# HpWang-whu/YOHO

Hardware: AMD Instinct MI355X
Metric: keypoints/sec (5000 kp x60 rot desc+YOHO-O) (higher is better)
Workload: dtype fp16x2 split (2^-22-accurate products, fp32 accumulate); 1 GPU

## Files before the change

### yoho_amd/csrc/gemmf2.hip

```cpp
#include <hip/hip_runtime.h>
#include <cstdlib>
#include <cstring>
#include "common.h"
#include "gemmf.h"

namespace yoho {

constexpr int F2_BUF = 24576;
constexpr int F2_LDS = 3 * F2_BUF;
constexpr int F3_BUF = 32768;
constexpr int F3_LDS = 3 * F3_BUF;

struct Frags2 {
    uintx4 ah[4], al[4], bh[2], bl[2];
};

template <int LO, int R>
__device__ __forceinline__ void read_frag2(const char* pa, const char* pb, Frags2& f) {
    if constexpr (R < 4) f.al[R] = *reinterpret_cast<const uintx4*>(pa + 8192 + R * 512);
    else if constexpr (R < 6) f.bh[R - 4] = *reinterpret_cast<const uintx4*>(pb + (R - 4) * 512);
    else if constexpr (R < 10) f.ah[R - 6] = *reinterpret_cast<const uintx4*>(pa + (R - 6) * 512);
    else f.bl[R - 10] = *reinterpret_cast<const uintx4*>(pb + LO + (R - 10) * 512);
}
template <int LO>
__device__ __forceinline__ void read_frags2(const char* pa, const char* pb, Frags2& f) {
    sfor<0, 12>([&](auto rc) { read_frag2<LO, decltype(rc)::value>(pa, pb, f); });
}

struct Dma2 {
    static constexpr int NP = 6, LO = 4096;
    int la, lb, w;
    __device__ __forceinline__ Dma2(int w_, int lane) : la(w_ * 1024 + lane * 16), lb((w_ >> 1) * 4096 + (w_ & 1) * 1024 + lane * 16), w(w_) {}
    template <int U>
    __device__ __forceinline__ void piece(const char* srcA, const char* srcB, char* buf) const {
        if constexpr (U < 4) {
            constexpr int plane = U >> 1, kg = U & 1;
            __builtin_amdgcn_global_load_lds((gptr_t)(srcA + plane * 16384 + kg * 4096 + la), (lptr_t)(buf + plane * 8192 + kg * 4096 + w * 1024), 16, 0, 0);
        } else {
            constexpr int plane = U - 4;
            __builtin_amdgcn_global_load_lds((gptr_t)(srcB + plane * 16384 + lb), (lptr_t)(buf + 16384 + plane * 4096 + (w >> 1) * 2048 + (w & 1) * 1024), 16, 0, 0);
        }
    }
};
struct Dma3 {
    static constexpr int NP = 4, LO = 8192;
    int la, ldst;
    __device__ __forceinline__ Dma3(int w8, int lane) : la(w8 * 1024 + lane * 16), ldst(w8 * 1024) {}
    template <int U>
    __device__ __forceinline__ void piece(const char* srcA, const char* srcB, char* buf) const {
        constexpr int plane = U & 1;
        if constexpr (U < 2) __builtin_amdgcn_global_load_lds((gptr_t)(srcA + plane * 16384 + la), (lptr_t)(buf + plane * 8192 + ldst), 16, 0, 0);
        else __builtin_amdgcn_global_load_lds((gptr_t)(srcB + plane * 16384 + la), (lptr_t)(buf + 16384 + plane * 8192 + ldst), 16, 0, 0);
    }
};
template <typename Dma>
__device__ __forceinline__ void dma_step(const Dma& dm, const char* srcA, const char* srcB, char* buf) {
    sfor<0, Dma::NP>([&](auto uc) { dm.template piece<decltype(uc)::value>(srcA, srcB, buf); });
}

template <bool DMA, typename Dma>
__device__ __forceinline__ void step2(const Dma& dm, const Frags2& f, floatx16 (&acc)[4][2], const char* ra, const char* rb, Frags2& nf,
                                      const char* srcA, const char* srcB, char* dmabuf) {
    sfor<0, 8>([&](auto gc) {
        constexpr int g = decltype(gc)::value;
        acc[g >> 1][g & 1] = mfma_h(f.al[g >> 1], f.bh[g & 1], acc[g >> 1][g & 1]);
        read_frag2<Dma::LO, g>(ra, rb, nf);
        __builtin_amdgcn_sched_barrier(0);
    });
    sfor<0, 8>([&](auto gc) {
        constexpr int g = decltype(gc)::value;
        acc[g >> 1][g & 1] = mfma_h(f.ah[g >> 1], f.bl[g & 1], acc[g >> 1][g & 1]);
        if constexpr (g < 4) read_frag2<Dma::LO, 8 + g>(ra, rb, nf);
        else if constexpr (DMA) dm.template piece<g - 4>(srcA, srcB, dmabuf);
        __builtin_amdgcn_sched_barrier(0);
    });
    sfor<0, 8>([&](auto gc) {
        constexpr int g = decltype(gc)::value;
        acc[g >> 1][g & 1] = mfma_h(f.ah[g >> 1], f.bh[g & 1], acc[g >> 1][g & 1]);
        if constexpr (DMA && 4 + g < Dma::NP) dm.template piece<4 + g>(srcA, srcB, dmabuf);
        __builtin_amdgcn_sched_barrier(0);
    });
}

__host__ __device__ inline bool fg2_map(const FGemmArgs& a, int xcd, int slot, bool contiguous, int& t, int& local, int& r) {
    int cnt[NIR_ORD], ru[NIR_ORD];
    for (int u = 0; u < NIR_ORD; ++u) {
        ru[u] = (xcd + a.rot[u]) & 7;
        cnt[u] = a.NT[u] > ru[u] ? ((a.NT[u] - 1 - ru[u]) / 8 + 1) * a.MT[u] * 2 : 0;
    }
    const int L = cnt[0], S = cnt[1] + cnt[2] + cnt[3] + cnt[4];
    int list, idx;
    if (contiguous) { list = slot < L ? 0 : 1; idx = slot < L ? slot : slot - L; }
    else {
        const int P = L < S ? L : S;
        if (slot < 2 * P) { list = slot & 1; idx = slot >> 1; }
        else { list = L > S ? 0 : 1; idx = P + (slot - 2 * P); }
    }
    if (list == 0) {
        if (idx >= L) return false;
        t = 0; local = idx; r = ru[0];
        return true;
    }
    for (int u = 1; u < NIR_ORD; ++u) {
        if (idx < cnt[u]) { t = u; local = idx; r = ru[u]; return true; }
        idx -= cnt[u];
    }
    return false;
}

__device__ __forceinline__ size_t step_off(int ks) { return (size_t)(ks >> 1) * FG_STAGE + (size_t)(ks & 1) * 8192; }

template <int BUF, typename Dma>
__device__ __forceinline__ void ring_prologue(int KT, Dma&& dma) {
    dma(0, 0);
    dma(1, BUF);
    if (KT > 2) dma(2, 2 * BUF);
}

template <int BUF, int INFLIGHT, typename F, typename Step>
__device__ __forceinline__ void ring_pipelined(char* smem, const char* Ag, const char* Bg, int KT, int lane_a, int lane_b, F& P, Step&& step) {
    F Q;
    asm volatile("s_waitcnt lgkmcnt(0)" ::: "memory");
    __builtin_amdgcn_s_barrier();
    __builtin_amdgcn_sched_barrier(0);
    int cur = 0, nxt = BUF;
    int s = 0;
    auto run = [&](auto dma, const F& f, F& nf) {
        if constexpr (decltype(dma)::value) {
            step(dma, f, nf, smem + nxt + lane_a, smem + nxt + lane_b, uniform_ptr(Ag + step_off(s + 3)), uniform_ptr(Bg + step_off(s + 3)), smem + cur);
            asm volatile("s_waitcnt vmcnt(%0) lgkmcnt(0)" ::"n"(INFLIGHT) : "memory");
        } else {
            step(dma, f, nf, smem + nxt + lane_a, smem + nxt + lane_b, nullptr, nullptr, nullptr);
            asm volatile("s_waitcnt vmcnt(0) lgkmcnt(0)" ::: "memory");
        }
        __builtin_amdgcn_s_barrier();
        __builtin_amdgcn_sched_barrier(0);
        cur = nxt; nxt = nxt == 2 * BUF ? 0 : nxt + BUF; ++s;
    };
    constexpr std::true_type dma;
    constexpr std::false_type nodma;
    while (s + 4 < KT) {
        run(dma, P, Q);
        run(dma, Q, P);
    }
    if (KT >= 4) {
        run(dma, P, Q);
        run(nodma, Q, P);
    }
    run(nodma, P, Q);
    step(nodma, Q, P, smem + cur + lane_a, smem + cur + lane_b, nullptr, nullptr, nullptr);
}

template <int BUF, typename Dma>
__device__ __forceinline__ void ring_pipelined_idle(int KT, Dma&& dma) {
    __builtin_amdgcn_s_barrier();
    for (int s = 0; s + 1 < KT; ++s) {
        if (s + 3 < KT) dma(s + 3, (s % 3) * BUF);
        asm volatile("s_waitcnt vmcnt(0)" ::: "memory");
        __builtin_amdgcn_s_barrier();
    }
}

__global__ __launch_bounds__(256, 2) void fgemm2_kernel(FGemmArgs a, int flags) {
    extern __shared__ __attribute__((aligned(16))) char smem[];
    const int tid = threadIdx.x, lane = tid & 63;
    const int w = __builtin_amdgcn_readfirstlane(tid >> 6);
    int t = 0, local = 0, r = 0;
    if (!fg2_map(a, blockIdx.x & 7, blockIdx.x >> 3, (flags & F2_MIX) == 0, t, local, r)) return;
    const int d = a.dim[t];
    const int MT = a.MT[t], KS = d * a.cin / 32, KT = 2 * KS;
    const int nh = local & 1, pair = local >> 1;
    const int cg = pair / MT, mtile = pair - cg * MT;
    const int ntile = r + 8 * cg;
    const char* Ag = a.A + a.a_off[t] + (size_t)mtile * KS * FG_STAGE;
    const char* Bg = a.B + a.b_off[t] + (size_t)ntile * KS * FG_STAGE + nh * 2048;
    const int wm = w >> 1, wn = w & 1;
    const Dma2 dm(w, lane);
    const int lane_a = (lane >> 5) * 4096 + (wm * 128 + (lane & 31)) * 16;
    const int lane_b = 16384 + (lane >> 5) * 2048 + (wn * 64 + (lane & 31)) * 16;

    floatx16 acc[4][2];
    zero_acc(acc);
    auto dma = [&](int st, int buf) { dma_step(dm, Ag + step_off(st), Bg + step_off(st), smem + buf); };
    ring_prologue<F2_BUF>(KT, dma);
    const int row0 = mtile * 256 + wm * 128, colbase = ntile * 256 + nh * 128 + wn * 64;
    const bool rows_live = row0 < d * a.cout;
    const int jidx = colbase / a.kppad, kp0 = colbase - jidx * a.kppad, qbase = a.qbase[t];
    if ((flags & EPI_RES) && rows_live) residual_start(acc, row0, kp0, jidx, d, qbase, a.res, a.descale, a.cout, a.nT32, lane);
    asm volatile("s_waitcnt vmcnt(0)" ::: "memory");
    __builtin_amdgcn_s_barrier();
    if (!rows_live) return ring_pipelined_idle<F2_BUF>(KT, dma);

    Frags2 P;
    read_frags2<Dma2::LO>(smem + lane_a, smem + lane_b, P);
    ring_pipelined<F2_BUF, 6>(smem, Ag, Bg, KT, lane_a, lane_b, P,
        [&](auto dmac, const Frags2& f, Frags2& nf, const char* ra, const char* rb, const char* srcA, const char* srcB, char* buf) {
            step2<decltype(dmac)::value>(dm, f, acc, ra, rb, nf, srcA, srcB, buf);
        });
    coef_epilogue(acc, row0, kp0, jidx, d, qbase, a.out, a.bias, a.descale, a.cout, a.nT32, a.rflag, lane, flags);
}

struct Wave3 {
    int wm, wn, nh, lane_a, lane_b;
    Dma3 dm;
    __device__ __forceinline__ Wave3(int w8, int lane) : wm((w8 & 3) >> 1), wn(w8 & 1), nh(w8 >> 2), dm(w8, lane) {
        lane_a = (lane >> 5) * 4096 + (wm * 128 + (lane & 31)) * 16;
        lane_b = 16384 + (lane >> 5) * 4096 + (nh * 128 + wn * 64 + (lane & 31)) * 16;
    }
};

__global__ __launch_bounds__(512, 2) void fgemm3_kernel(FGemmArgs a, int flags) {
    extern __shared__ __attribute__((aligned(16))) char smem[];
    const int tid = threadIdx.x, lane = tid & 63;
    const Wave3 wv(__builtin_amdgcn_readfirstlane(tid >> 6), lane);
    int t = 0, local = 0, r = 0;
    if (!fg3_map(a, blockIdx.x & 7, blockIdx.x >> 3, t, local, r)) return;
    const int d = a.dim[t];
    const int MT = a.MT[t], KS = d * a.cin / 32, KT = 2 * KS;
    const int cg = local / MT, mtile = local - cg * MT;
    const int ntile = r + 8 * cg;
    const char* Ag = a.A + a.a_off[t] + (size_t)mtile * KS * FG_STAGE;
    const char* Bg = a.B + a.b_off[t] + (size_t)ntile * KS * FG_STAGE;

    floatx16 acc[4][2];
    zero_acc(acc);
    auto dma = [&](int st, int buf) { dma_step(wv.dm, Ag + step_off(st), Bg + step_off(st), smem + buf); };
    ring_prologue<F3_BUF>(KT, dma);
    const int row0 = mtile * 256 + wv.wm * 128, colbase = ntile * 256 + wv.nh * 128 + wv.wn * 64;
    const bool rows_live = row0 < d * a.cout;
    const int jidx = colbase / a.kppad, kp0 = colbase - jidx * a.kppad, qbase = a.qbase[t];
    if ((flags & EPI_RES) && rows_live) residual_start(acc, row0, kp0, jidx, d, qbase, a.res, a.descale, a.cout, a.nT32, lane);
    asm volatile("s_waitcnt vmcnt(0)" ::: "memory");
    __builtin_amdgcn_s_barrier();
    if (!rows_live) return ring_pipelined_idle<F3_BUF>(KT, dma);

    Frags2 P;
    read_frags2<Dma3::LO>(smem + wv.lane_a, smem + wv.lane_b, P);
    ring_pipelined<F3_BUF, 4>(smem, Ag, Bg, KT, wv.lane_a, wv.lane_b, P,
        [&](auto dmac, const Frags2& f, Frags2& nf, const char* ra, const char* rb, const char* srcA, const char* srcB, char* buf) {
            step2<decltype(dmac)::value>(wv.dm, f, acc, ra, rb, nf, srcA, srcB, buf);
        });
    coef_epilogue(acc, row0, kp0, jidx, d, qbase, a.out, a.bias, a.descale, a.cout, a.nT32, a.rflag, lane, flags);
}

constexpr int F3K_BUF = 2 * FG_STAGE;
constexpr int F3K_LDS = 2 * F3K_BUF;

struct Dma3k {
    static constexpr int NP = 8;
    int la, ldst;
    __device__ __forceinline__ Dma3k(int w8, int lane) : la(w8 * 1024 + lane * 16), ldst(w8 * 1024) {}
    template <int U>
    __device__ __forceinline__ void piece(const char* srcA, const char* srcB, char* buf) const {
        constexpr int q = (U & 3) * 8192;
        if constexpr (U < 4) __builtin_amdgcn_global_load_lds((gptr_t)(srcA + q + la), (lptr_t)(buf + q + ldst), 16, 0, 0);
        else __builtin_amdgcn_global_load_lds((gptr_t)(srcB + q + la), (lptr_t)(buf + FG_STAGE + q + ldst), 16, 0, 0);
    }
};
struct FragsA32 { uintx4 al, ah; };
struct FragsB32 { uintx4 bh[4], bl[4]; };

template <int R>
__device__ __forceinline__ void read_open32(const char* pa, const char* pb, FragsA32& a0, FragsB32& b) {
    if constexpr (R == 0) a0.al = *reinterpret_cast<const uintx4*>(pa + 16384);
    else if constexpr (R < 5) b.bh[R - 1] = *reinterpret_cast<const uintx4*>(pb + (R - 1) * 256);
    else if constexpr (R == 5) a0.ah = *reinterpret_cast<const uintx4*>(pa);
    else b.bl[R - 6] = *reinterpret_cast<const uintx4*>(pb + 16384 + (R - 6) * 256);
}

template <bool DMA>
__device__ __forceinline__ void step32(const Dma3k& dm, floatx4 (&acc)[8][4], FragsA32 (&fa)[2], const FragsB32& b, FragsB32& nb, const char* pa,
                                       const char* npa, const char* npb, const char* srcA, const char* srcB, char* dmabuf) {
    sfor<0, 7>([&](auto ic) {
        constexpr int i = decltype(ic)::value;
        row_products32(acc[i], fa[i & 1].al, fa[i & 1].ah, b.bh, b.bl, [&](auto mc) {
            constexpr int m = decltype(mc)::value;
            if constexpr (m == 1) fa[(i + 1) & 1].al = *reinterpret_cast<const uintx4*>(pa + 16384 + (i + 1) * 256);
            if constexpr (m == 2) fa[(i + 1) & 1].ah = *reinterpret_cast<const uintx4*>(pa + (i + 1) * 256);
        });
    });
    asm volatile("s_waitcnt vmcnt(0) lgkmcnt(0)" ::: "memory");
    __builtin_amdgcn_s_barrier();
    __builtin_amdgcn_sched_barrier(0);
    row_products32(acc[7], fa[1].al, fa[1].ah, b.bh, b.bl, [&](auto mc) {
        constexpr int m = decltype(mc)::value;
        if constexpr (m < 5) {
            read_open32<2 * m>(npa, npb, fa[0], nb);
            read_open32<2 * m + 1>(npa, npb, fa[0], nb);
        }
        if constexpr (DMA && m >= 4) dm.template piece<m - 4>(srcA, srcB, dmabuf);
    });
}

__global__ __launch_bounds__(512, 2) void fgemm3k_kernel(FGemmArgs a, int flags) {
    extern __shared__ __attribute__((aligned(16))) char smem[];
    const int tid = threadIdx.x, lane = tid & 63;
    const int w8 = __builtin_amdgcn_readfirstlane(tid >> 6);
    int t = 0, local = 0, r = 0;
    if (!fg3_map(a, blockIdx.x & 7, blockIdx.x >> 3, t, local, r)) return;
    const int d = a.dim[t];
    const int MT = a.MT[t], KS = d * a.cin / 32;
    const int cg = local / MT, mtile = local - cg * MT;
    const int ntile = r + 8 * cg;
    const char* Ag = a.A + a.a_off[t] + (size_t)mtile * KS * FG_STAGE;
    const char* Bg = a.B + a.b_off[t] + (size_t)ntile * KS * FG_STAGE;
    const int wm = (w8 & 3) >> 1, wn = w8 & 1, nh = w8 >> 2;
    const Dma3k dm(w8, lane);
    const int lane_a = (lane >> 4) * 4096 + (wm * 128 + (lane & 15)) * 16;
    const int lane_b = FG_STAGE + (lane >> 4) * 4096 + (nh * 128 + wn * 64 + (lane & 15)) * 16;

    floatx4 acc[8][4];
    zero_acc(acc);
    auto dma = [&](int st, int buf) {
        const char* sa = uniform_ptr(Ag + (size_t)st * FG_STAGE);
        const char* sb = uniform_ptr(Bg + (size_t)st * FG_STAGE);
        sfor<0, Dma3k::NP>([&](auto uc) { dm.template piece<decltype(uc)::value>(sa, sb, smem + buf); });
    };
    dma(0, 0);
    if (KS > 1) dma(1, F3K_BUF);
    const int row0 = mtile * 256 + wm * 128, colbase = ntile * 256 + nh * 128 + wn * 64;
    const bool rows_live = row0 < d * a.cout;
    const int jidx = colbase / a.kppad, kp0 = colbase - jidx * a.kppad, qbase = a.qbase[t];
    if ((flags & EPI_RES) && rows_live) residual_start(acc, row0, kp0, jidx, d, qbase, a.res, a.descale, a.cout, a.nT32, lane);
    asm volatile("s_waitcnt vmcnt(0)" ::: "memory");
    __builtin_amdgcn_s_barrier();
    if (!rows_live) {
        for (int s = 0; s < KS; ++s) {
            asm volatile("s_waitcnt vmcnt(0)" ::: "memory");
            __builtin_amdgcn_s_barrier();
            if (s + 2 < KS) dma(s + 2, (s & 1) * F3K_BUF);
        }
        asm volatile("s_waitcnt vmcnt(0)" ::: "memory");
        return;
    }

    FragsA32 fa[2];
    FragsB32 P, Q;
    sfor<0, 10>([&](auto rc) { read_open32<decltype(rc)::value>(smem + lane_a, smem + lane_b, fa[0], P); });
    int s = 0, cur = 0;
    auto run = [&](auto dmac, const FragsB32& b, FragsB32& nb) {
        const int nxt = cur ^ F3K_BUF;
        if constexpr (decltype(dmac)::value)
            step32<true>(dm, acc, fa, b, nb, smem + cur + lane_a, smem + nxt + lane_a, smem + nxt + lane_b, uniform_ptr(Ag + (size_t)(s + 2) * FG_STAGE),
                         uniform_ptr(Bg + (size_t)(s + 2) * FG_STAGE), smem + cur);
        else
            step32<false>(dm, acc, fa, b, nb, smem + cur + lane_a, smem + nxt + lane_a, smem + nxt + lane_b, nullptr, nullptr, nullptr);
        cur = nxt; ++s;
    };
    constexpr std::true_type dmay;
    constexpr std::false_type dman;
    while (s + 2 < KS) {
        run(dmay, P, Q);
        run(dmay, Q, P);
    }
    run(dman, P, Q);
    run(dman, Q, P);
    coef_epilogue(acc, row0, kp0, jidx, d, qbase, a.out, a.bias, a.descale, a.cout, a.nT32, a.rflag, lane, flags);
}

constexpr int F2K_BUF = FG_STAGE + FG_STAGE / 2;
constexpr int F2K_LDS = 2 * F2K_BUF;

__global__ __launch_bounds__(256, 1) void fgemm2k_kernel(FGemmArgs a, int flags) {
    extern __shared__ __attribute__((aligned(16))) char smem[];
    const int tid = threadIdx.x, lane = tid & 63;
    const int w = __builtin_amdgcn_readfirstlane(tid >> 6);
    int t = 0, local = 0, r = 0;
    if (!fg2_map(a, blockIdx.x & 7, blockIdx.x >> 3, (flags & F2_MIX) == 0, t, local, r)) return;
    const int d = a.dim[t];
    const int MT = a.MT[t], KS = d * a.cin / 32;
    const int nh = local & 1, pair = local >> 1;
    const int cg = pair / MT, mtile = pair - cg * MT;
    const int ntile = r + 8 * cg;
    const char* Ag = a.A + a.a_off[t] + (size_t)mtile * KS * FG_STAGE;
    const char* Bg = a.B + a.b_off[t] + (size_t)ntile * KS * FG_STAGE + nh * 2048;
    const int wm = w >> 1, wn = w & 1;
    const int lane_a = (lane >> 4) * 4096 + (wm * 128 + (lane & 15)) * 16;
    const int lane_b = FG_STAGE + (lane >> 4) * 2048 + (wn * 64 + (lane & 15)) * 16;

    floatx4 acc[8][4];
    zero_acc(acc);
    auto dma = [&](int st, int buf) {
        const char* sa = uniform_ptr(Ag + (size_t)st * FG_STAGE) + lane * 16;
        const char* sb = uniform_ptr(Bg + (size_t)st * FG_STAGE) + lane * 16;
#pragma unroll
        for (int k = 0; k < 8; ++k) __builtin_amdgcn_global_load_lds((gptr_t)(sa + (k * 4 + w) * 1024), (lptr_t)(smem + buf + (k * 4 + w) * 1024), 16, 0, 0);
#pragma unroll
        for (int k = 0; k < 4; ++k) {
            const int pb = w * 4 + k, u = pb >> 1, part = pb & 1;
            __builtin_amdgcn_global_load_lds((gptr_t)(sb + u * 4096 + part * 1024), (lptr_t)(smem + buf + FG_STAGE + u * 2048 + part * 1024), 16, 0, 0);
        }
    };
    dma(0, 0);
    if (KS > 1) dma(1, F2K_BUF);
    const int row0 = mtile * 256 + wm * 128, colbase = ntile * 256 + nh * 128 + wn * 64;
    const bool rows_live = row0 < d * a.cout;
    const int jidx = colbase / a.kppad, kp0 = colbase - jidx * a.kppad, qbase = a.qbase[t];
    if ((flags & EPI_RES) && rows_live) residual_start(acc, row0, kp0, jidx, d, qbase, a.res, a.descale, a.cout, a.nT32, lane);
    asm volatile("s_waitcnt vmcnt(0)" ::: "memory");
    __builtin_amdgcn_s_barrier();
    for (int s = 0; s < KS; ++s) {
        const int cur = (s & 1) * F2K_BUF;
        if (rows_live) stage32_plain<FG_STAGE / 4>(acc, smem + cur + lane_a, smem + cur + lane_b);
        asm volatile("s_waitcnt vmcnt(0) lgkmcnt(0)" ::: "memory");
        __builtin_amdgcn_s_barrier();
        __builtin_amdgcn_sched_barrier(0);
        if (s + 2 < KS) dma(s + 2, cur);
    }
    if (rows_live) coef_epilogue(acc, row0, kp0, jidx, d, qbase, a.out, a.bias, a.descale, a.cout, a.nT32, a.rflag, lane, flags);
}

typedef int intx8 __attribute__((ext_vector_type(8)));
typedef short shortx2 __attribute__((ext_vector_type(2)));
typedef _Float16 halfx2 __attribute__((ext_vector_type(2)));
struct Frags8 {
    intx8 a[4], b[2];
};
struct C8Scales {
    float ah = 4.f, al = 4.f / 2048.f, bh = 1.f, bl = 1.f;
    int mfma_b = 127;
    C8Scales() = default;
    __device__ __forceinline__ explicit C8Scales(const unsigned* amax) {
        const unsigned amax_bits = __builtin_amdgcn_readfirstlane(*amax);
        int kexp = (int)(amax_bits >> 23) - 127 - 7;
        kexp = kexp < -60 ? -60 : (kexp > 9 ? 9 : kexp);
        bh = __uint_as_float((unsigned)(kexp + 127) << 23); bl = __uint_as_float((unsigned)(kexp - 11 + 127) << 23);
        mfma_b = 127 + kexp;
    }
};
struct Int2 { int x, y; };
__device__ __forceinline__ Int2 frag_to_fp8(uintx4 f, float scale) {
    union { unsigned u; halfx2 h; } p0, p1, p2, p3;
    p0.u = f[0]; p1.u = f[1]; p2.u = f[2]; p3.u = f[3];
    shortx2 r = {0, 0}, q = {0, 0};
    r = __builtin_amdgcn_cvt_scalef32_pk_fp8_f16(r, p0.h, scale, false);
    r = __builtin_amdgcn_cvt_scalef32_pk_fp8_f16(r, p1.h, scale, true);
    q = __builtin_amdgcn_cvt_scalef32_pk_fp8_f16(q, p2.h, scale, false);
    q = __builtin_amdgcn_cvt_scalef32_pk_fp8_f16(q, p3.h, scale, true);
    Int2 o;
    __builtin_memcpy(&o.x, &r, 4);
    __builtin_memcpy(&o.y, &q, 4);
    return o;
}

template <int PAR>
__device__ __forceinline__ void step3c(const Frags2& f, floatx16 (&acc)[4][2], Frags8& c8, const C8Scales& sc) {
#pragma unroll
    for (int i = 0; i < 4; ++i)
#pragma unroll
        for (int j = 0; j < 2; ++j) acc[i][j] = mfma_h(f.ah[i], f.bh[j], acc[i][j]);
#pragma unroll
    for (int i = 0; i < 4; ++i)
#pragma unroll
        for (int e = 0; e < 4; ++e) c8.a[i][4 * PAR + e] = (int)f.al[i][e];
#pragma unroll
    for (int j = 0; j < 2; ++j) {
        const Int2 l = frag_to_fp8(f.bl[j], sc.bl), h = frag_to_fp8(f.bh[j], sc.bh);
        c8.b[j][4 * PAR] = l.x; c8.b[j][4 * PAR + 1] = l.y; c8.b[j][4 * PAR + 2] = h.x; c8.b[j][4 * PAR + 3] = h.y;
    }
    if constexpr (PAR == 1) {
#pragma unroll
        for (int i = 0; i < 4; ++i)
#pragma unroll
            for (int j = 0; j < 2; ++j)
                acc[i][j] = __builtin_amdgcn_mfma_scale_f32_32x32x64_f8f6f4(c8.a[i], c8.b[j], acc[i][j], 0, 0, 0, 127 + 2 - 11, 0, sc.mfma_b);
    }
}

template <bool FP8, typename BSrc>
__device__ __forceinline__ void ring_plain(floatx16 (&acc)[4][2], char* smem, const Wave3& wv, const char* Ag, BSrc&& bsrc, int KT, bool rows_live,
                                           const C8Scales& sc) {
    Frags8 c8;
    if constexpr (FP8) {
#pragma unroll
        for (int i = 0; i < 4; ++i)
#pragma unroll
            for (int e = 0; e < 8; ++e) c8.a[i][e] = 0;
#pragma unroll
        for (int j = 0; j < 2; ++j)
#pragma unroll
            for (int e = 0; e < 8; ++e) c8.b[j][e] = 0;
    }
    int cur = 0, stg = 2 * F3_BUF;
    int s = 0;
    auto stage = [&] {
        const int s2 = s + 2 < KT ? s + 2 : KT - 1;
        dma_step(wv.dm, uniform_ptr(Ag + step_off(s2)), uniform_ptr(bsrc(s2)), smem + stg);
    };
    auto rotate = [&] { stg = cur; cur = cur == 2 * F3_BUF ? 0 : cur + F3_BUF; ++s; };
    auto one_step = [&](auto parity) {
        asm volatile("s_waitcnt vmcnt(4) lgkmcnt(0)" ::: "memory");
        __builtin_amdgcn_s_barrier();
        __builtin_amdgcn_sched_barrier(0);
        stage();
        Frags2 f;
        read_frags2<Dma3::LO>(smem + cur + wv.lane_a, smem + cur + wv.lane_b, f);
        if constexpr (FP8) step3c<decltype(parity)::value>(f, acc, c8, sc);
        else {
#pragma unroll
            for (int i = 0; i < 4; ++i)
#pragma unroll
                for (int j = 0; j < 2; ++j) acc[i][j] = mfma_h(f.al[i], f.bh[j], acc[i][j]);
#pragma unroll
            for (int i = 0; i < 4; ++i)
#pragma unroll
                for (int j = 0; j < 2; ++j) acc[i][j] = mfma_h(f.ah[i], f.bl[j], acc[i][j]);
#pragma unroll
            for (int i = 0; i < 4; ++i)
#pragma unroll
                for (int j = 0; j < 2; ++j) acc[i][j] = mfma_h(f.ah[i], f.bh[j], acc[i][j]);
        }
        rotate();
    };
    if (rows_live) {
        for (int it = 0; it < KT; it += 2) {
            one_step(std::integral_constant<int, 0>{});
            one_step(std::integral_constant<int, 1>{});
        }
    } else {
        for (int it = 0; it < KT; ++it) {
            asm volatile("s_waitcnt vmcnt(4) lgkmcnt(0)" ::: "memory");
            __builtin_amdgcn_s_barrier();
            stage();
            rotate();
        }
    }
    asm volatile("s_waitcnt vmcnt(0)" ::: "memory");
}

__global__ __launch_bounds__(512, 2) void fgemm3c_kernel(FGemmArgs a, int flags) {
    extern __shared__ __attribute__((aligned(16))) char smem[];
    const int tid = threadIdx.x, lane = tid & 63;
    const Wave3 wv(__builtin_amdgcn_readfirstlane(tid >> 6), lane);
    int t = 0, local = 0, r = 0;
    if (!fg3_map(a, blockIdx.x & 7, blockIdx.x >> 3, t, local, r)) return;
    const int d = a.dim[t];
    const int MT = a.MT[t], KS = d * a.cin / 32, KT = 2 * KS;
    const int cg = local / MT, mtile = local - cg * MT;
    const int ntile = r + 8 * cg;
    const char* Ag = a.A + a.a_off[t] + (size_t)mtile * KS * FG_STAGE;
    const char* Bg = a.B + a.b_off[t] + (size_t)ntile * KS * FG_STAGE;

    floatx16 acc[4][2];
    zero_acc(acc);
    const C8Scales sc(a.amax);
    dma_step(wv.dm, Ag, Bg, smem);
    dma_step(wv.dm, Ag + step_off(1), Bg + step_off(1), smem + F3_BUF);
    const int row0 = mtile * 256 + wv.wm * 128, colbase = ntile * 256 + wv.nh * 128 + wv.wn * 64;
    const bool rows_live = row0 < d * a.cout;
    const int jidx = colbase / a.kppad, kp0 = colbase - jidx * a.kppad, qbase = a.qbase[t];
    if ((flags & EPI_RES) && rows_live) residual_start(acc, row0, kp0, jidx, d, qbase, a.res, a.descale, a.cout, a.nT32, lane);
    asm volatile("s_waitcnt vmcnt(0)" ::: "memory");
    __builtin_amdgcn_s_barrier();

    ring_plain<true>(acc, smem, wv, Ag, [&](int s) { return Bg + step_off(s); }, KT, rows_live, sc);
    if (rows_live) coef_epilogue(acc, row0, kp0, jidx, d, qbase, a.out, a.bias, a.descale, a.cout, a.nT32, a.rflag, lane, flags);
}

struct CGemmArgs {
    const char* A;
    const char* B;
    const float* bias;
    const float* bn_s;
    const float* bn_t;
    char* out;
    int NTm, MT, KSt, ntap, nj, nslot, c8out, nT32, nTiles16;
    float descale;
    int* rflag;
    const unsigned* amax;
    unsigned char slot[13 * 13];
    unsigned char outg[16];
};

__device__ __forceinline__ void cg_split_pair(float x0, float x1, unsigned& hi, unsigned& lo) {
    typedef float f2 __attribute__((ext_vector_type(2)));
    f2 x;
    x.x = x0; x.y = x1;
    const halfx2 h = __builtin_convertvector(x, halfx2);
    const f2 r = x - __builtin_convertvector(h, f2);
    const halfx2 l = __builtin_convertvector(r, halfx2);
    __builtin_memcpy(&hi, &h, 4);
    __builtin_memcpy(&lo, &l, 4);
}

template <bool FP8>
__global__ __launch_bounds__(512, 2) void cgemm_kernel(CGemmArgs a) {
    extern __shared__ __attribute__((aligned(16))) char smem[];
    __shared__ int tapoff[16];
    const int tid = threadIdx.x, lane = tid & 63;
    const Wave3 wv(__builtin_amdgcn_readfirstlane(tid >> 6), lane);
    const int xcd = blockIdx.x & 7, slot_ = blockIdx.x >> 3;
    const int ct = xcd + 8 * (slot_ / a.MT), mtile = slot_ % a.MT;
    if (ct >= a.nj * a.NTm) return;
    const int j = ct / a.NTm, mt = ct - j * a.NTm;
    const int SPT = 2 * a.KSt;
    const int KT = a.ntap * SPT;
    if (tid < 16) tapoff[tid] = tid < a.ntap ? (int)a.slot[j * 13 + tid] : 0;
    const char* Ag = a.A + (size_t)mtile * (KT / 2) * FG_STAGE;
    const char* Bt = a.B + (size_t)mt * a.nslot * a.KSt * FG_STAGE;
    __syncthreads();
    auto bsrc = [&](int s) -> const char* {
        const int tap = s / SPT, within = s - tap * SPT;
        const int sl = __builtin_amdgcn_readfirstlane(tapoff[tap]);
        return Bt + (size_t)sl * a.KSt * FG_STAGE + step_off(within);
    };

    floatx16 acc[4][2];
    zero_acc(acc);
    C8Scales sc;
    if constexpr (FP8) sc = C8Scales(a.amax);
    dma_step(wv.dm, Ag, uniform_ptr(bsrc(0)), smem);
    dma_step(wv.dm, Ag + step_off(1), uniform_ptr(bsrc(1)), smem + F3_BUF);
    asm volatile("s_waitcnt vmcnt(0)" ::: "memory");
    __builtin_amdgcn_s_barrier();

    ring_plain<FP8>(acc, smem, wv, Ag, bsrc, KT, true, sc);

    const int half = lane >> 5, c32 = lane & 31;
    const int g = a.outg[j];
    unsigned top = 0u;
#pragma unroll
    for (int bi = 0; bi < 2; ++bi) {
        const int m = mt * 256 + wv.nh * 128 + wv.wn * 64 + bi * 32 + c32;
        if ((m >> 5) >= a.nT32 || (m >> 4) >= a.nTiles16) continue;
#pragma unroll
        for (int ai = 0; ai < 4; ++ai) {
#pragma unroll
            for (int q4 = 0; q4 < 4; ++q4) {
                const int o = mtile * 256 + wv.wm * 128 + ai * 32 + q4 * 8 + half * 4;
                const floatx4 b4 = *reinterpret_cast<const floatx4*>(a.bias + o);
                const floatx4 s4 = *reinterpret_cast<const floatx4*>(a.bn_s + o);
                const floatx4 t4 = *reinterpret_cast<const floatx4*>(a.bn_t + o);
                float y[4];
#pragma unroll
                for (int e = 0; e < 4; ++e) {
                    const float v = acc[ai][bi][4 * q4 + e] * a.descale + b4[e];
                    y[e] = fmaxf(v * s4[e] + t4[e], 0.f) * H2_ASCALE;
                    top = max(top, __float_as_uint(y[e]) & 0x7FFFFFFFu);
                }
                unsigned h0, l0, h1, l1;
                cg_split_pair(y[0], y[1], h0, l0);
                cg_split_pair(y[2], y[3], h1, l1);
                char* dst = a.out + (((size_t)(m >> 4) * a.c8out + (o >> 3)) * 2) * 15360 + g * 256 + (m & 15) * 16 + half * 8;
                *reinterpret_cast<uint2*>(dst) = uint2{h0, h1};
                *reinterpret_cast<uint2*>(dst + 15360) = uint2{l0, l1};
            }
        }
    }
    note_range_bits(a.rflag, top, FP16_MAX);
}

int cgemm_init() {
    HIPCHK(hipFuncSetAttribute(reinterpret_cast<const void*>(&cgemm_kernel<true>), hipFuncAttributeMaxDynamicSharedMemorySize, F3_LDS));
    HIPCHK(hipFuncSetAttribute(reinterpret_cast<const void*>(&cgemm_kernel<false>), hipFuncAttributeMaxDynamicSharedMemorySize, F3_LDS));
    return 0;
}

int launch_cgemm(const Layer& L, const char* Bstages, int nslot, const unsigned char* slot, const unsigned char* outg, int nT32, int nTiles16,
                 char* out, hipStream_t s, int* rflag, const unsigned* amax) {
    const bool fp8 = amax != nullptr;
    if (!(fp8 ? L.wcg8 : L.wcg) || L.cin % 32 || L.cout % 256) { set_error("cgemm: needs the cone-GEMM weight pack, cin %% 32 == 0, cout %% 256 == 0"); return YOHO_EINVAL; }
    if (nT32 == 0) return 0;
    CGemmArgs a;
    a.A = reinterpret_cast<const char*>(fp8 ? L.wcg8 : L.wcg); a.B = Bstages; a.bias = L.bias; a.bn_s = L.bn_s; a.bn_t = L.bn_t; a.out = out;
    a.NTm = (nT32 + 7) / 8; a.MT = L.cout / 256; a.KSt = L.cin / 32; a.ntap = 13; a.nj = 13; a.nslot = nslot; a.c8out = L.cout / 8;
    a.nT32 = nT32; a.nTiles16 = nTiles16; a.descale = L.wcg_descale; a.rflag = rflag; a.amax = amax;
    std::memcpy(a.slot, slot, 169);
    std::memset(a.outg, 0, 16);
    std::memcpy(a.outg, outg, 13);
    const int CT = a.nj * a.NTm;
    const int grid = 8 * ((CT + 7) / 8) * a.MT;
    if (fp8) hipLaunchKernelGGL(cgemm_kernel<true>, dim3(grid), dim3(512), F3_LDS, s, a);
    else hipLaunchKernelGGL(cgemm_kernel<false>, dim3(grid), dim3(512), F3_LDS, s, a);
    HIPCHK(hipGetLastError());
    return 0;
}

struct Frags3s {
    uintx4 ah[5], al[5], bh, bl;
};

template <int R>
__device__ __forceinline__ void read_frag3s(const char* pa, const char* pb, Frags3s& f) {
    if constexpr (R < 5) f.al[R] = *reinterpret_cast<const uintx4*>(pa + 8192 + R * 512);
    else if constexpr (R == 5) f.bh = *reinterpret_cast<const uintx4*>(pb);
    else if constexpr (R < 11) f.ah[R - 6] = *reinterpret_cast<const uintx4*>(pa + (R - 6) * 512);
    else f.bl = *reinterpret_cast<const uintx4*>(pb + 8192);
}

template <bool DMA, int D>
__device__ __forceinline__ void step3s(const Frags3s& f, floatx16 (&acc)[5][1], const char* ra, const char* rb, Frags3s& nf,
                                       const char* srcA, const char* srcB, char* dmabuf, const Dma3& dm) {
    sfor<0, 5>([&](auto gc) {
        constexpr int g = decltype(gc)::value;
        if constexpr (g < D) acc[g][0] = mfma_h(f.al[g], f.bh, acc[g][0]);
        if constexpr (g < D) read_frag3s<g>(ra, rb, nf);
        if constexpr (g == 4) read_frag3s<5>(ra, rb, nf);
        __builtin_amdgcn_sched_barrier(0);
    });
    sfor<0, 5>([&](auto gc) {
        constexpr int g = decltype(gc)::value;
        if constexpr (g < D) acc[g][0] = mfma_h(f.ah[g], f.bl, acc[g][0]);
        if constexpr (g < D) read_frag3s<6 + g>(ra, rb, nf);
        if constexpr (g == 4) read_frag3s<11>(ra, rb, nf);
        __builtin_amdgcn_sched_barrier(0);
    });
    sfor<0, 5>([&](auto gc) {
        constexpr int g = decltype(gc)::value;
        if constexpr (g < D) acc[g][0] = mfma_h(f.ah[g], f.bh, acc[g][0]);
        if constexpr (DMA && g < 4) dm.template piece<g>(srcA, srcB, dmabuf);
        __builtin_amdgcn_sched_barrier(0);
    });
}

template <int D>
__device__ __forceinline__ void fgemm3s_kloop(floatx16 (&acc)[5][1], char* smem, const char* Ag, const char* Bg, int KT, const Dma3& dm, int lane_a, int lane_b) {
    Frags3s P;
    sfor<0, 12>([&](auto rc) {
        constexpr int R = decltype(rc)::value;
        if constexpr (R == 5 || R == 11 || (R < 5 && R < D) || (R > 5 && R < 11 && R - 6 < D)) read_frag3s<R>(smem + lane_a, smem + lane_b, P);
    });
    ring_pipelined<F3_BUF, 4>(smem, Ag, Bg, KT, lane_a, lane_b, P,
        [&](auto dmac, const Frags3s& f, Frags3s& nf, const char* ra, const char* rb, const char* srcA, const char* srcB, char* buf) {
            step3s<decltype(dmac)::value, D>(f, acc, ra, rb, nf, srcA, srcB, buf, dm);
        });
}

__global__ __launch_bounds__(512, 2) void fgemm3s_kernel(FGemmArgs a, int flags) {
    extern __shared__ __attribute__((aligned(16))) char smem[];
    const int tid = threadIdx.x, lane = tid & 63;
    const int w8 = __builtin_amdgcn_readfirstlane(tid >> 6);
    int t = 0, local = 0, r = 0;
    if (!fg3_map(a, blockIdx.x & 7, blockIdx.x >> 3, t, local, r)) return;
    const int d = a.dim[t];
    const int KS = d * a.cin / 32, KT = 2 * KS;
    const int ntile = r + 8 * local;
    const char* Ag = a.A + a.a_off[t];
    const char* Bg = a.B + a.b_off[t] + (size_t)ntile * KS * FG_STAGE;
    const Dma3 dm(w8, lane);
    const int lane_a = (lane >> 5) * 4096 + (lane & 31) * 16;
    const int lane_b = 16384 + (lane >> 5) * 4096 + (w8 * 32 + (lane & 31)) * 16;

    floatx16 acc[5][1];
    zero_acc(acc);
    ring_prologue<F3_BUF>(KT, [&](int st, int buf) { dma_step(dm, uniform_ptr(Ag + step_off(st)), uniform_ptr(Bg + step_off(st)), smem + buf); });
    asm volatile("s_waitcnt vmcnt(0)" ::: "memory");
    __builtin_amdgcn_s_barrier();

    switch (d) {
        case 1: fgemm3s_kloop<1>(acc, smem, Ag, Bg, KT, dm, lane_a, lane_b); break;
        case 3: fgemm3s_kloop<3>(acc, smem, Ag, Bg, KT, dm, lane_a, lane_b); break;
        case 4: fgemm3s_kloop<4>(acc, smem, Ag, Bg, KT, dm, lane_a, lane_b); break;
        default: fgemm3s_kloop<5>(acc, smem, Ag, Bg, KT, dm, lane_a, lane_b); break;
    }
    const int colbase = ntile * 256 + w8 * 32;
    const int jidx = colbase / a.kppad, kp0 = colbase - jidx * a.kppad;
    coef_epilogue(acc, 0, kp0, jidx, d, a.qbase[t], a.out, a.bias, a.descale, 32, a.nT32, a.rflag, lane, flags & F2_NOSTORE);
}

int fgemm3_init() {
    HIPCHK(hipFuncSetAttribute(reinterpret_cast<const void*>(&fgemm3_kernel), hipFuncAttributeMaxDynamicSharedMemorySize, F3_LDS));
    HIPCHK(hipFuncSetAttribute(reinterpret_cast<const void*>(&fgemm3s_kernel), hipFuncAttributeMaxDynamicSharedMemorySize, F3_LDS));
    HIPCHK(hipFuncSetAttribute(reinterpret_cast<const void*>(&fgemm3c_kernel), hipFuncAttributeMaxDynamicSharedMemorySize, F3_LDS));
    HIPCHK(hipFuncSetAttribute(reinterpret_cast<const void*>(&fgemm3k_kernel), hipFuncAttributeMaxDynamicSharedMemorySize, F3K_LDS));
    return 0;
}

int launch_fgemm3(const FGemmArgs& a, int flags, hipStream_t s) {
    if (const char* dbg = experiment_env("YOHO_FGEMM_DEBUG")) {
        if (std::strstr(dbg, "nostore")) flags |= F2_NOSTORE;
        if (std::strstr(dbg, "sc1")) flags |= F2_ST_SC1;
        if (std::strstr(dbg, "stnt")) flags |= F2_ST_NT;
    }
    const int tot = fgemm_grid(a, 1);
    static const bool small_ok = [] { const char* e = experiment_env("YOHO_FGEMM_DEBUG"); return !(e && std::strstr(e, "nosmall")); }();
    if (small_ok && a.cout == 32 && !(flags & EPI_RES)) hipLaunchKernelGGL(fgemm3s_kernel, dim3(tot), dim3(512), F3_LDS, s, a, flags);
    else if (a.amax) hipLaunchKernelGGL(fgemm3c_kernel, dim3(tot), dim3(512), F3_LDS, s, a, flags);
    else if (flags & F2_K32) hipLaunchKernelGGL(fgemm3k_kernel, dim3(tot), dim3(512), F3K_LDS, s, a, flags);
    else hipLaunchKernelGGL(fgemm3_kernel, dim3(tot), dim3(512), F3_LDS, s, a, flags);
    HIPCHK(hipGetLastError());
    return 0;
}

int fgemm2_init() {
    HIPCHK(hipFuncSetAttribute(reinterpret_cast<const void*>(&fgemm2_kernel), hipFuncAttributeMaxDynamicSharedMemorySize, F2_LDS));
    HIPCHK(hipFuncSetAttribute(reinterpret_cast<const void*>(&fgemm2k_kernel), hipFuncAttributeMaxDynamicSharedMemorySize, F2K_LDS));
    return fgemm3_init();
}

int launch_fgemm2(const FGemmArgs& a, int flags, hipStream_t s) {
    if (const char* dbg = experiment_env("YOHO_FGEMM_DEBUG")) {
        if (std::strstr(dbg, "nostore")) flags |= F2_NOSTORE;
        if (std::strstr(dbg, "mix")) flags |= F2_MIX;
        if (std::strstr(dbg, "sc1")) flags |= F2_ST_SC1;
        if (std::strstr(dbg, "nt")) flags |= F2_ST_NT;
        if (std::strstr(dbg, "sparse4")) flags |= F2_SPARSE4;
        if (std::strstr(dbg, "sparse16")) flags |= F2_SPARSE16;
    }
    if (flags & F2_K32) hipLaunchKernelGGL(fgemm2k_kernel, dim3(fgemm_grid(a, 2)), dim3(256), F2K_LDS, s, a, flags);
    else hipLaunchKernelGGL(fgemm2_kernel, dim3(fgemm_grid(a, 2)), dim3(256), F2_LDS, s, a, flags);
    HIPCHK(hipGetLastError());
    return 0;
}

}
```

Before: 1.800 million keypoints/s.

## Move K32 fgemm stage barrier mid-stage and split DMA across stage halves

Reworks the K=32 split-fp16 GEMM pipeline so the stage-handoff barrier sits after row MROW rather than at the end of each stage. Reads of the next stage's fragments and the global-to-LDS DMA pieces are spread over the remaining rows, and part of the next A tile is prefetched at the head of the stage. The aim is to hide barrier and load latency behind MFMA work instead of draining everything at the stage end. This adds a second barrier per stage and more complex buffer-reuse ordering, which risks LDS races or extra stalls. The old schedule is kept under an experiments flag.

```diff
diff --git a/yoho_amd/csrc/gemmf2.hip b/yoho_amd/csrc/gemmf2.hip
--- a/yoho_amd/csrc/gemmf2.hip
+++ b/yoho_amd/csrc/gemmf2.hip
@@ -268,9 +268,54 @@
     else b.bl[R - 6] = *reinterpret_cast<const uintx4*>(pb + 16384 + (R - 6) * 256);
 }
 
+constexpr int F3K_MROW = 4;
+
+template <int MROW, bool HEAD, bool DMA, bool NEXT>
+__device__ __forceinline__ void step32(const Dma3k& dm, floatx4 (&acc)[8][4], FragsA32 (&fa)[2], const FragsB32& b, FragsB32& nb, const char* pa,
+                                       const char* npa, const char* npb, const char* headA, char* headbuf, const char* srcA, const char* srcB,
+                                       char* dmabuf) {
+    static_assert(MROW >= 3 && MROW <= 5, "M in the middle of the stage");
+    constexpr int NRB = 7 - MROW, PER = (8 + NRB - 1) / NRB;
+    constexpr int NRD = 6 - MROW, DSTEP = NRD >= 2 ? 2 : 1;
+    sfor<0, 8>([&](auto ic) {
+        constexpr int i = decltype(ic)::value;
+        row_products32(acc[i], fa[i & 1].al, fa[i & 1].ah, b.bh, b.bl, [&](auto mc) {
+            constexpr int m = decltype(mc)::value;
+            if constexpr (NEXT && i == MROW + 1 && m == 0) {
+                asm volatile("s_waitcnt vmcnt(0) lgkmcnt(0)" ::: "memory");
+                __builtin_amdgcn_s_barrier();
+            }
+            if constexpr (DMA && i == 7 && m == 0) {
+                asm volatile("s_waitcnt lgkmcnt(0)" ::: "memory");
+                __builtin_amdgcn_s_barrier();
+            }
+            if constexpr (i < 7) {
+                if constexpr (m == 1) fa[(i + 1) & 1].al = *reinterpret_cast<const uintx4*>(pa + 16384 + (i + 1) * 256);
+                if constexpr (m == 2) fa[(i + 1) & 1].ah = *reinterpret_cast<const uintx4*>(pa + (i + 1) * 256);
+            } else if constexpr (NEXT) {
+                if constexpr (m == 1) read_open32<0>(npa, npb, fa[0], nb);
+                if constexpr (m == 2) read_open32<5>(npa, npb, fa[0], nb);
+            }
+            if constexpr (NEXT && i > MROW && m >= 3 && m < 3 + PER) {
+                constexpr int k = (i - MROW - 1) * PER + m - 3;
+                if constexpr (k < 8) read_open32<(k < 4 ? 1 : 2) + k>(npa, npb, fa[0], nb);
+            }
+            if constexpr (DMA && i > MROW && i < 7 && m >= 7 && (m - 7) % DSTEP == 0) {
+                constexpr int k = i - MROW - 1 + NRD * ((m - 7) / DSTEP);
+                if constexpr (k < 4) dm.template piece<4 + k>(srcA, srcB, dmabuf);
+            }
+            if constexpr (DMA && i == 7 && m == 7) dm.template piece<0>(srcA, srcB, dmabuf);
+            if constexpr (DMA && i == 7 && m == 10) dm.template piece<1>(srcA, srcB, dmabuf);
+            if constexpr (HEAD && i == 0 && m == 4) dm.template piece<2>(headA, nullptr, headbuf);
+            if constexpr (HEAD && i == 0 && m == 8) dm.template piece<3>(headA, nullptr, headbuf);
+        });
+    });
+}
+
+#ifdef YOHO_EXPERIMENTS
 template <bool DMA>
-__device__ __forceinline__ void step32(const Dma3k& dm, floatx4 (&acc)[8][4], FragsA32 (&fa)[2], const FragsB32& b, FragsB32& nb, const char* pa,
-                                       const char* npa, const char* npb, const char* srcA, const char* srcB, char* dmabuf) {
+__device__ __forceinline__ void step32a(const Dma3k& dm, floatx4 (&acc)[8][4], FragsA32 (&fa)[2], const FragsB32& b, FragsB32& nb, const char* pa,
+                                        const char* npa, const char* npb, const char* srcA, const char* srcB, char* dmabuf) {
     sfor<0, 7>([&](auto ic) {
         constexpr int i = decltype(ic)::value;
         row_products32(acc[i], fa[i & 1].al, fa[i & 1].ah, b.bh, b.bl, [&](auto mc) {
@@ -291,7 +336,9 @@
         if constexpr (DMA && m >= 4) dm.template piece<m - 4>(srcA, srcB, dmabuf);
     });
 }
-
+#endif
+
+template <int MROW>
 __global__ __launch_bounds__(512, 2) void fgemm3k_kernel(FGemmArgs a, int flags) {
     extern __shared__ __attribute__((aligned(16))) char smem[];
     const int tid = threadIdx.x, lane = tid & 63;
@@ -311,50 +358,92 @@
 
     floatx4 acc[8][4];
     zero_acc(acc);
-    auto dma = [&](int st, int buf) {
+    auto dma = [&](auto u0, auto u1, int st, int buf) {
         const char* sa = uniform_ptr(Ag + (size_t)st * FG_STAGE);
         const char* sb = uniform_ptr(Bg + (size_t)st * FG_STAGE);
-        sfor<0, Dma3k::NP>([&](auto uc) { dm.template piece<decltype(uc)::value>(sa, sb, smem + buf); });
+        sfor<decltype(u0)::value, decltype(u1)::value>([&](auto uc) { dm.template piece<decltype(uc)::value>(sa, sb, smem + buf); });
     };
-    dma(0, 0);
-    if (KS > 1) dma(1, F3K_BUF);
+    constexpr std::integral_constant<int, 0> u0;
+    constexpr std::integral_constant<int, 2> u2;
+    constexpr std::integral_constant<int, 4> u4;
+    constexpr std::integral_constant<int, 8> u8;
+    dma(u0, u8, 0, 0);
+    dma(u4, u8, 1, F3K_BUF);
+    if constexpr (MROW != 0) dma(u0, u2, 1, F3K_BUF);
+    else dma(u0, u4, 1, F3K_BUF);
     const int row0 = mtile * 256 + wm * 128, colbase = ntile * 256 + nh * 128 + wn * 64;
     const bool rows_live = row0 < d * a.cout;
     const int jidx = colbase / a.kppad, kp0 = colbase - jidx * a.kppad, qbase = a.qbase[t];
     if ((flags & EPI_RES) && rows_live) residual_start(acc, row0, kp0, jidx, d, qbase, a.res, a.descale, a.cout, a.nT32, lane);
     asm volatile("s_waitcnt vmcnt(0)" ::: "memory");
     __builtin_amdgcn_s_barrier();
+    constexpr std::true_type yes;
+    constexpr std::false_type no;
+    FragsA32 fa[2];
+    FragsB32 P, Q;
+    int s = 0, cur = 0;
+#ifdef YOHO_EXPERIMENTS
+    if constexpr (MROW == 0) {
+        if (!rows_live) {
+            for (; s < KS; ++s) {
+                asm volatile("s_waitcnt vmcnt(0)" ::: "memory");
+                __builtin_amdgcn_s_barrier();
+                if (s + 2 < KS) dma(u0, u8, s + 2, (s & 1) * F3K_BUF);
+            }
+            asm volatile("s_waitcnt vmcnt(0)" ::: "memory");
+            return;
+        }
+        sfor<0, 10>([&](auto rc) { read_open32<decltype(rc)::value>(smem + lane_a, smem + lane_b, fa[0], P); });
+        auto run = [&](auto dmac, const FragsB32& b, FragsB32& nb) {
+            const int nxt = cur ^ F3K_BUF;
+            if constexpr (decltype(dmac)::value)
+                step32a<true>(dm, acc, fa, b, nb, smem + cur + lane_a, smem + nxt + lane_a, smem + nxt + lane_b, uniform_ptr(Ag + (size_t)(s + 2) * FG_STAGE),
+                              uniform_ptr(Bg + (size_t)(s + 2) * FG_STAGE), smem + cur);
+            else
+                step32a<false>(dm, acc, fa, b, nb, smem + cur + lane_a, smem + nxt + lane_a, smem + nxt + lane_b, nullptr, nullptr, nullptr);
+            cur = nxt; ++s;
+        };
+        while (s + 2 < KS) {
+            run(yes, P, Q);
+            run(yes, Q, P);
+        }
+        run(no, P, Q);
+        run(no, Q, P);
+        coef_epilogue(acc, row0, kp0, jidx, d, qbase, a.out, a.bias, a.descale, a.cout, a.nT32, a.rflag, lane, flags);
+        return;
+    }
+#endif
+    constexpr int MR = MROW ? MROW : F3K_MROW;
     if (!rows_live) {
-        for (int s = 0; s < KS; ++s) {
+        for (; s + 1 < KS; ++s, cur ^= F3K_BUF) {
+            dma(u2, u4, s + 1, cur ^ F3K_BUF);
             asm volatile("s_waitcnt vmcnt(0)" ::: "memory");
             __builtin_amdgcn_s_barrier();
-            if (s + 2 < KS) dma(s + 2, (s & 1) * F3K_BUF);
-        }
-        asm volatile("s_waitcnt vmcnt(0)" ::: "memory");
+            if (s + 2 < KS) {
+                dma(u4, u8, s + 2, cur);
+                __builtin_amdgcn_s_barrier();
+                dma(u0, u2, s + 2, cur);
+            }
+        }
         return;
     }
 
-    FragsA32 fa[2];
-    FragsB32 P, Q;
     sfor<0, 10>([&](auto rc) { read_open32<decltype(rc)::value>(smem + lane_a, smem + lane_b, fa[0], P); });
-    int s = 0, cur = 0;
-    auto run = [&](auto dmac, const FragsB32& b, FragsB32& nb) {
+    auto run = [&](auto head, auto dmac, auto next, const FragsB32& b, FragsB32& nb) {
         const int nxt = cur ^ F3K_BUF;
-        if constexpr (decltype(dmac)::value)
-            step32<true>(dm, acc, fa, b, nb, smem + cur + lane_a, smem + nxt + lane_a, smem + nxt + lane_b, uniform_ptr(Ag + (size_t)(s + 2) * FG_STAGE),
-                         uniform_ptr(Bg + (size_t)(s + 2) * FG_STAGE), smem + cur);
-        else
-            step32<false>(dm, acc, fa, b, nb, smem + cur + lane_a, smem + nxt + lane_a, smem + nxt + lane_b, nullptr, nullptr, nullptr);
+        constexpr bool H = decltype(head)::value, D = decltype(dmac)::value;
+        step32<MR, H, D, decltype(next)::value>(dm, acc, fa, b, nb, smem + cur + lane_a, smem + nxt + lane_a, smem + nxt + lane_b,
+                                                H ? uniform_ptr(Ag + (size_t)(s + 1) * FG_STAGE) : nullptr, smem + nxt,
+                                                D ? uniform_ptr(Ag + (size_t)(s + 2) * FG_STAGE) : nullptr,
+                                                D ? uniform_ptr(Bg + (size_t)(s + 2) * FG_STAGE) : nullptr, smem + cur);
         cur = nxt; ++s;
     };
-    constexpr std::true_type dmay;
-    constexpr std::false_type dman;
     while (s + 2 < KS) {
-        run(dmay, P, Q);
-        run(dmay, Q, P);
-    }
-    run(dman, P, Q);
-    run(dman, Q, P);
+        run(yes, yes, yes, P, Q);
+        run(yes, yes, yes, Q, P);
+    }
+    run(yes, no, yes, P, Q);
+    run(no, no, no, Q, P);
     coef_epilogue(acc, row0, kp0, jidx, d, qbase, a.out, a.bias, a.descale, a.cout, a.nT32, a.rflag, lane, flags);
 }
 
@@ -762,7 +851,13 @@
     HIPCHK(hipFuncSetAttribute(reinterpret_cast<const void*>(&fgemm3_kernel), hipFuncAttributeMaxDynamicSharedMemorySize, F3_LDS));
     HIPCHK(hipFuncSetAttribute(reinterpret_cast<const void*>(&fgemm3s_kernel), hipFuncAttributeMaxDynamicSharedMemorySize, F3_LDS));
     HIPCHK(hipFuncSetAttribute(reinterpret_cast<const void*>(&fgemm3c_kernel), hipFuncAttributeMaxDynamicSharedMemorySize, F3_LDS));
-    HIPCHK(hipFuncSetAttribute(reinterpret_cast<const void*>(&fgemm3k_kernel), hipFuncAttributeMaxDynamicSharedMemorySize, F3K_LDS));
+    HIPCHK(hipFuncSetAttribute(reinterpret_cast<const void*>(&fgemm3k_kernel<F3K_MROW>), hipFuncAttributeMaxDynamicSharedMemorySize, F3K_LDS));
+#ifdef YOHO_EXPERIMENTS
+    HIPCHK(hipFuncSetAttribute(reinterpret_cast<const void*>(&fgemm3k_kernel<0>), hipFuncAttributeMaxDynamicSharedMemorySize, F3K_LDS));
+    HIPCHK(hipFuncSetAttribute(reinterpret_cast<const void*>(&fgemm3k_kernel<3>), hipFuncAttributeMaxDynamicSharedMemorySize, F3K_LDS));
+    HIPCHK(hipFuncSetAttribute(reinterpret_cast<const void*>(&fgemm3k_kernel<4>), hipFuncAttributeMaxDynamicSharedMemorySize, F3K_LDS));
+    HIPCHK(hipFuncSetAttribute(reinterpret_cast<const void*>(&fgemm3k_kernel<5>), hipFuncAttributeMaxDynamicSharedMemorySize, F3K_LDS));
+#endif
     return 0;
 }
 
@@ -776,7 +871,18 @@
     static const bool small_ok = [] { const char* e = experiment_env("YOHO_FGEMM_DEBUG"); return !(e && std::strstr(e, "nosmall")); }();
     if (small_ok && a.cout == 32 && !(flags & EPI_RES)) hipLaunchKernelGGL(fgemm3s_kernel, dim3(tot), dim3(512), F3_LDS, s, a, flags);
     else if (a.amax) hipLaunchKernelGGL(fgemm3c_kernel, dim3(tot), dim3(512), F3_LDS, s, a, flags);
-    else if (flags & F2_K32) hipLaunchKernelGGL(fgemm3k_kernel, dim3(tot), dim3(512), F3K_LDS, s, a, flags);
+    else if (flags & F2_K32) {
+#ifdef YOHO_EXPERIMENTS
+        const char* dbg = experiment_env("YOHO_FGEMM_DEBUG");
+        const int mrow = !dbg ? F3K_MROW : std::strstr(dbg, "k32a") ? 0 : std::strstr(dbg, "k32m3") ? 3 : std::strstr(dbg, "k32m4") ? 4 : std::strstr(dbg, "k32m5") ? 5 : F3K_MROW;
+        if (mrow == 0) hipLaunchKernelGGL(fgemm3k_kernel<0>, dim3(tot), dim3(512), F3K_LDS, s, a, flags);
+        else if (mrow == 3) hipLaunchKernelGGL(fgemm3k_kernel<3>, dim3(tot), dim3(512), F3K_LDS, s, a, flags);
+        else if (mrow == 5) hipLaunchKernelGGL(fgemm3k_kernel<5>, dim3(tot), dim3(512), F3K_LDS, s, a, flags);
+        else hipLaunchKernelGGL(fgemm3k_kernel<4>, dim3(tot), dim3(512), F3K_LDS, s, a, flags);
+#else
+        hipLaunchKernelGGL(fgemm3k_kernel<F3K_MROW>, dim3(tot), dim3(512), F3K_LDS, s, a, flags);
+#endif
+    }
     else hipLaunchKernelGGL(fgemm3_kernel, dim3(tot), dim3(512), F3_LDS, s, a, flags);
     HIPCHK(hipGetLastError());
     return 0;
```

Measured after the change: 1.804 million keypoints/s, median of 6. No clear change (+0.3%).
